# DarylFernandes99/custom-yolo-implmentation

Measured on AMD Instinct MI355X. Metric: images/sec (640x640 bf16), higher is better.
Workload: dtype bf16; 1 GPU; preset s (width 32..512, depth 1) 640x640 train step (fwd+DFL/QFL loss+bwd+grad sync+AdamW), COCO-80 synthetic, 32 img/GPU; global_batch=32, parallelism=dp1, hip_graph=True, optimizer_in_graph=True, deterministic_mode=False

## Files before the change

### custom-yolo-implmentation_amd/csrc/loss.hip

```cpp
#include "common.h"

namespace {

constexpr int REG = 16;
constexpr float QEPS = 1e-12f;

struct LossDims {
    int N, A, nc;
    float lambda_dfl, lambda_cls;
};

template <typename T>
__device__ __forceinline__ void decode_block(const LossDims& d, int block, const T* __restrict__ preds, const T* __restrict__ anchors,
                                             const T* __restrict__ strides, float4* __restrict__ pbox) {
    long i = block * (long)blockDim.x + threadIdx.x;
    if (i >= (long)d.N * d.A) return;
    int a = (int)(i % d.A);
    long n = i / d.A;
    const T* p = preds + n * (long)(4 * REG + d.nc) * d.A + a;
    float e[4];
#pragma unroll
    for (int s = 0; s < 4; ++s) {
        float x[REG], mx = -INFINITY;
#pragma unroll
        for (int b = 0; b < REG; ++b) { x[b] = to_f<T>(p[(long)(s * REG + b) * d.A]); mx = fmaxf(mx, x[b]); }
        float sum = 0.f;
#pragma unroll
        for (int b = 0; b < REG; ++b) { x[b] = expf(x[b] - mx); sum += x[b]; }
        float ex = 0.f;
#pragma unroll
        for (int b = 0; b < REG; ++b) ex += (x[b] / sum) * (float)b;
        e[s] = ex;
    }
    float ax = to_f<T>(anchors[a]), ay = to_f<T>(anchors[d.A + a]), st = to_f<T>(strides[a]);
    float x1 = (ax - e[0]) * st, y1 = (ay - e[1]) * st, x2 = (ax + e[2]) * st, y2 = (ay + e[3]) * st;
    pbox[i] = make_float4((x1 + x2) / 2.f, (y1 + y2) / 2.f, x2 - x1, y2 - y1);
}

__device__ __forceinline__ int assign_wave(int A, const float4* __restrict__ pb, const float* __restrict__ gt, int j, int lane) {
    const float gx = gt[j * 5 + 0], gy = gt[j * 5 + 1];
    const float an = __fadd_rn(__fmul_rn(gx, gx), __fmul_rn(gy, gy));
    const float m2x = -2.f * gx, m2y = -2.f * gy;
    float best = INFINITY;
    int bi = 0x7fffffff;
    auto consider = [&](int a, const float4& b) {
        float bn = __fadd_rn(__fmul_rn(b.x, b.x), __fmul_rn(b.y, b.y));
        float acc = __fmul_rn(m2x, b.x);
        acc = __fmaf_rn(m2y, b.y, acc);
        acc = __fadd_rn(an, acc);
        acc = __fadd_rn(bn, acc);
        float dist = __fsqrt_rn(fmaxf(acc, 0.f));
// ... 37 lines not shown
    float dpos = -2.f * om * ls + om * om / (s + QEPS);
    float dneg = 2.f * s * l1 - s * s / (1.f - s + QEPS);
    dx = -(t * dpos + (1.f - t) * dneg) * s * om;
}

__device__ __forceinline__ void qfl_elem0(float x, float& val, float& dx) {
    float s = sigm(x);
    float l1 = logf(1.f - s + QEPS);
    float om = 1.f - s;
    val = -(s * s * l1);
    float dneg = 2.f * s * l1 - s * s / (1.f - s + QEPS);
    dx = -dneg * s * om;
}

template <typename T, int V>
__device__ __forceinline__ void dense_block(const LossDims& d, int block, int nblk, const T* __restrict__ preds, T* __restrict__ dpreds,
                                            float coef, double* __restrict__ partial, const float* __restrict__ grad_scale) {
    __shared__ float red[4];
    if (grad_scale) coef *= *grad_scale;
    const int Cp = 4 * REG + d.nc;
    const int P = d.nc * (d.A / V), Z = 4 * REG * (d.A / V);
    const int nthr = nblk * 256, gtid = block * 256 + threadIdx.x;
    constexpr int U = 4;
    float lsum = 0.f;
    const long per_img = (long)Cp * d.A;
    for (long i0 = gtid; i0 < (long)d.N * P; i0 += (long)nthr * U) {
        pack_t<T, V> raw[U];
        long eo[U];
#pragma unroll
        for (int u = 0; u < U; ++u) {
            const long idx = i0 + (long)u * nthr;
            const long ic = idx < (long)d.N * P ? idx : i0;
            const int n = (int)(ic / P), off = (int)(ic - (long)n * P);
            eo[u] = n * per_img + (long)4 * REG * d.A + (long)off * V;
            raw[u] = load_raw<T, V>(preds + eo[u]);
        }
#pragma unroll
        for (int u = 0; u < U; ++u) {
            if (i0 + (long)u * nthr >= (long)d.N * P) break;
            float x[V], g[V];
            unpack<T, V>(raw[u], x);
#pragma unroll
            for (int e = 0; e < V; ++e) {
                float v, dx;
                qfl_elem0(x[e], v, dx);
                lsum += v;
                g[e] = dx * coef;
            }
            if (dpreds) store_pack<T, V>(dpreds + eo[u], g);
        }
    }
    if (dpreds) {
        float z[V];
#pragma unroll
        for (int k = 0; k < V; ++k) z[k] = 0.f;
        for (long idx = gtid; idx < (long)d.N * Z; idx += nthr) {
            const int n = (int)(idx / Z), off = (int)(idx - (long)n * Z);
            store_pack<T, V>(dpreds + n * per_img + (long)off * V, z);
        }
    }
    lsum = wave_sum(lsum);
    if ((threadIdx.x & 63) == 0) red[threadIdx.x >> 6] = lsum;
    __syncthreads();
    if (threadIdx.x == 0) partial[block] = (double)red[0] + red[1] + red[2] + red[3];
}

template <typename T, int V>
__global__ __launch_bounds__(256) void k_front(LossDims d, int DB, int nblk, const T* __restrict__ preds, const T* __restrict__ anchors,
                                               const T* __restrict__ strides, float4* __restrict__ pbox, T* __restrict__ dpreds,
                                               float coef, double* __restrict__ partial, const float* __restrict__ grad_scale,
                                               unsigned int* __restrict__ ticket) {
    if (blockIdx.x == 0 && threadIdx.x == 0) *ticket = 0u;
    if ((int)blockIdx.x < DB) decode_block<T>(d, blockIdx.x, preds, anchors, strides, pbox);
    else dense_block<T, V>(d, (int)blockIdx.x - DB, nblk, preds, dpreds, coef, partial, grad_scale);
}

__device__ void finish_scalars(const LossDims& d, const double* partial, int nblk, const double* img_dfl, const double* img_cls_fix,
                               float* __restrict__ out);

template <typename T>
__global__ __launch_bounds__(256) void k_back(LossDims d, const T* __restrict__ preds, T* __restrict__ dpreds,
                                              const T* __restrict__ anchors, const T* __restrict__ strides,
                                              const float4* __restrict__ pbox, const float* __restrict__ gt,
                                              const int* __restrict__ gt_off, const int* __restrict__ idx,
                                              double* __restrict__ img_dfl, double* __restrict__ img_cls_fix,
                                              const float* __restrict__ grad_scale, const double* __restrict__ partial, int nblk,
                                              unsigned int* __restrict__ ticket, float* __restrict__ out) {
    __shared__ double w_dfl[4], w_cls[4];
    __shared__ unsigned int my_ticket;
    const float gsc = grad_scale ? *grad_scale : 1.f;
    const int n = blockIdx.x, lane = threadIdx.x & 63, wave = threadIdx.x >> 6;
    const int g0 = gt_off[n], M = gt_off[n + 1] - g0;

    const int Cp = 4 * REG + d.nc;
    const T* pn = preds + (long)n * Cp * d.A;
    T* dn = dpreds ? dpreds + (long)n * Cp * d.A : nullptr;
    const int side = lane >> 4, bin = lane & 15;
    const float cdfl = d.lambda_dfl / (float)d.N * 0.25f / (float)(M > 0 ? M : 1);
    const float ccls = d.lambda_cls / (float)d.N / (float)d.A;
    double acc_dfl = 0.0, acc_cls = 0.0;

    constexpr int PF = 40;
    const float4* pbn = pbox + (long)n * d.A;
    float2 pf[PF];
#pragma unroll
    for (int u = 0; u < PF; ++u) {
        const int a = threadIdx.x + u * 256;
        pf[u] = (dn && a < d.A) ? *reinterpret_cast<const float2*>(pbn + a) : make_float2(0.f, 0.f);
    }

    for (int j = wave; j < M; j += 4) {
        const int a = idx[g0 + j];
        bool owner = true;
        for (int q = 0; q < j; ++q) owner &= (idx[g0 + q] != a);
        if (!owner) continue;
        float x = to_f<T>(pn[(long)lane * d.A + a]);
        float mx = x;
#pragma unroll
        for (int o = 8; o > 0; o >>= 1) mx = fmaxf(mx, __shfl_xor(mx, o, 64));
        float ex = expf(x - mx), sum = ex;
#pragma unroll
        for (int o = 8; o > 0; o >>= 1) sum += __shfl_xor(sum, o, 64);
        float p = ex / sum, lse = mx + logf(sum);
        float ev = p * (float)bin;
#pragma unroll
        for (int o = 8; o > 0; o >>= 1) ev += __shfl_xor(ev, o, 64);
        const float ax = to_f<T>(anchors[a]), ay = to_f<T>(anchors[d.A + a]), st = to_f<T>(strides[a]);
        const float4 pb = pbox[(long)n * d.A + a];
        float gacc = 0.f;
        int winner = -1;
        for (int q = j; q < M; ++q)
// ... 12 lines not shown
            float contrib = (bin == lo ? wl * (lse - x) : 0.f) + (bin == lo + 1 ? wr * (lse - x) : 0.f);
            float side_loss = contrib;
#pragma unroll
            for (int o = 8; o > 0; o >>= 1) side_loss += __shfl_xor(side_loss, o, 64);
            float all_sides = side_loss + __shfl_xor(side_loss, 16, 64);
            all_sides += __shfl_xor(all_sides, 32, 64);
            if (lane == 0) acc_dfl += (double)all_sides * 0.25 / (double)M;
            gacc += cdfl * (p - (bin == lo ? wl : 0.f) - (bin == lo + 1 ? wr : 0.f));
            const float X1 = pb.x - pb.z / 2.f, Y1 = pb.y - pb.w / 2.f, X2 = pb.x + pb.z / 2.f, Y2 = pb.w + pb.y / 2.f;
            const float iwr = fminf(X2, gx2) - fmaxf(X1, gx1), ihr = fminf(Y2, gy2) - fmaxf(Y1, gy1);
            const float iw = fmaxf(iwr, 0.f), ih = fmaxf(ihr, 0.f);
            const float inter = iw * ih;
            const float a1 = (X2 - X1) * (Y2 - Y1), a2 = (gx2 - gx1) * (gy2 - gy1);
            const float den = a1 + a2 - inter + 1e-6f;
            const float iou = inter / den;
            const float xc = to_f<T>(pn[(long)(4 * REG + cls) * d.A + a]);
            const float sc = sigm(xc);
            const float omc = 1.f - sc;
            const float giou = ccls * -(omc * omc * logf(sc + QEPS) - sc * sc * logf(1.f - sc + QEPS));
            const float mX2 = X2 < gx2 ? 1.f : (X2 == gx2 ? 0.5f : 0.f), mX1 = X1 > gx1 ? 1.f : (X1 == gx1 ? 0.5f : 0.f);
            const float mY2 = Y2 < gy2 ? 1.f : (Y2 == gy2 ? 0.5f : 0.f), mY1 = Y1 > gy1 ? 1.f : (Y1 == gy1 ? 0.5f : 0.f);
            const float pw = iwr >= 0.f ? 1.f : 0.f, ph = ihr >= 0.f ? 1.f : 0.f;
            const float dI_X2 = ih * pw * mX2, dI_X1 = -ih * pw * mX1, dI_Y2 = iw * ph * mY2, dI_Y1 = -iw * ph * mY1;
            const float dA_X2 = (Y2 - Y1), dA_X1 = -(Y2 - Y1), dA_Y2 = (X2 - X1), dA_Y1 = -(X2 - X1);
            const float kI = 1.f / den + inter / (den * den), kA = inter / (den * den);
            const float dX1 = giou * (kI * dI_X1 - kA * dA_X1), dX2 = giou * (kI * dI_X2 - kA * dA_X2);
            const float dY1 = giou * (kI * dI_Y1 - kA * dA_Y1), dY2 = giou * (kI * dI_Y2 - kA * dA_Y2);
            const float dcx = dX1 + dX2, dw = (dX2 - dX1) / 2.f, dcy = dY1 + dY2 / 2.f, dh = dY2 - dY1 / 2.f;
            const float dx1 = dcx / 2.f - dw, dx2 = dcx / 2.f + dw, dy1 = dcy / 2.f - dh, dy2 = dcy / 2.f + dh;
            const float gs = side == 0 ? -st * dx1 : side == 1 ? -st * dy1 : side == 2 ? st * dx2 : st * dy2;
            gacc += gs * p * ((float)bin - ev);
            if (q == winner && lane == 0) {
                float v0, g0_, v1, g1_;
                qfl_elem(xc, 0.f, v0, g0_);
                qfl_elem(xc, iou, v1, g1_);
                acc_cls += (double)v1 - (double)v0;
                if (dn) dn[(long)(4 * REG + cls) * d.A + a] = from_f<T>(g1_ * ccls * gsc);
            }
        }
        if (dn) dn[(long)lane * d.A + a] = from_f<T>(gacc * gsc);
    }
    if (dn) {
        auto poison = [&](int a, float cx, float cy) {
            const bool bx = cx != cx, by = cy != cy;
            if (!(bx || by)) return;
            for (int c = 0; c < 4 * REG; ++c)
                if (((c >> 4) & 1) ? by : bx) dn[(long)c * d.A + a] = from_f<T>(NAN);
        };
#pragma unroll
        for (int u = 0; u < PF; ++u) poison(threadIdx.x + u * 256, pf[u].x, pf[u].y);
        for (int a = threadIdx.x + PF * 256; a < d.A; a += 256) poison(a, pbn[a].x, pbn[a].y);
    }
    if (lane == 0) { w_dfl[wave] = acc_dfl; w_cls[wave] = acc_cls; }
    __syncthreads();
    if (threadIdx.x == 0) {
        img_dfl[n] = w_dfl[0] + w_dfl[1] + w_dfl[2] + w_dfl[3];
        img_cls_fix[n] = w_cls[0] + w_cls[1] + w_cls[2] + w_cls[3];
        __threadfence();
        my_ticket = atomicAdd(ticket, 1u);
    }
    __syncthreads();
    if (my_ticket != (unsigned)d.N - 1u || wave != 0) return;
// ... 28 lines not shown
    double mean_cls = cls / (double)d.A / (double)d.N, mean_dfl = dfl / (double)d.N;
    out[0] = (float)(d.lambda_dfl * mean_dfl + d.lambda_cls * mean_cls);
    out[1] = (float)mean_dfl;
    out[2] = (float)mean_cls;
}

template <typename T>
__global__ void k_scale(T* __restrict__ x, long n, const float* __restrict__ s) {
    const float f = *s;
    for (long i = blockIdx.x * (long)blockDim.x + threadIdx.x; i < n; i += (long)gridDim.x * blockDim.x)
        x[i] = from_f<T>(to_f<T>(x[i]) * f);
}

constexpr int DENSE_BLOCKS = 2048;

}

extern "C" {

size_t yolo_loss_workspace_bytes(int N, int A, int G) {
    size_t b = (size_t)N * A * 16;
    b += ((size_t)(G > 0 ? G : 1) * 4 + 15) / 16 * 16;
    b += (size_t)(DENSE_BLOCKS + 2 * N) * 8;
    b += 16;
    return b;
}

int yolo_loss_dfl_qfl(const void* preds, const void* anchors, const void* strides, int dtype, int N, int nc, int A,
                      const float* gt, const int* gt_off, const int* gt_img, int G, float lambda_dfl,
                      float lambda_cls, void* dpreds, float* out, void* workspace, const float* grad_scale, hipStream_t st) {
    if (N < 1) return YOLO_ERR_ARG;
    LossDims d{N, A, nc, lambda_dfl, lambda_cls};
    char* ws = (char*)workspace;
    float4* pbox = (float4*)ws;
    ws += (size_t)N * A * 16;
    int* idx = (int*)ws;
    ws += ((size_t)(G > 0 ? G : 1) * 4 + 15) / 16 * 16;
    double* partial = (double*)ws;
    double* img_dfl = partial + DENSE_BLOCKS;
    double* img_fix = img_dfl + N;
    unsigned int* ticket = (unsigned int*)(img_fix + N);
    const long NA = (long)N * A;
    const long elems = NA * (64 + nc);
    const float coef = lambda_cls / (float)N / (float)A;
    const int DB = ceil_div(NA, 256);
    YOLO_DISPATCH_T(dtype, {
        constexpr int VV = vec_of<T>::N;
        bool vec = (A % VV == 0) && ((uintptr_t)preds % 16 == 0) && (!dpreds || (uintptr_t)dpreds % 16 == 0);
        int nblk = (int)((elems / (vec ? VV : 1) + 255) / 256);
        if (nblk > DENSE_BLOCKS) nblk = DENSE_BLOCKS;
        if (nblk < 1) nblk = 1;
        if (vec) hipLaunchKernelGGL((k_front<T, VV>), dim3(DB + nblk), dim3(256), 0, st, d, DB, nblk, (const T*)preds, (const T*)anchors,
                                    (const T*)strides, pbox, (T*)dpreds, coef, partial, grad_scale, ticket);
        else hipLaunchKernelGGL((k_front<T, 1>), dim3(DB + nblk), dim3(256), 0, st, d, DB, nblk, (const T*)preds, (const T*)anchors,
                                (const T*)strides, pbox, (T*)dpreds, coef, partial, grad_scale, ticket);
        if (G > 0) hipLaunchKernelGGL(k_assign, dim3(ceil_div(G, 4)), dim3(256), 0, st, A, pbox, gt, gt_img, gt_off, N, idx);
        hipLaunchKernelGGL((k_back<T>), dim3(N), dim3(256), 0, st, d, (const T*)preds, (T*)dpreds, (const T*)anchors,
                           (const T*)strides, pbox, gt, gt_off, idx, img_dfl, img_fix, grad_scale, partial, nblk, ticket, out);
    });
    return YOLO_LAUNCH_CHECK();
}

int yolo_scale_inplace(void* x, long n, int dtype, const float* scale_dev, hipStream_t st) {
    long b = (n + 255) / 256;
    if (b > 4096) b = 4096;
    if (b < 1) b = 1;
    YOLO_DISPATCH_T(dtype, hipLaunchKernelGGL((k_scale<T>), dim3((int)b), dim3(256), 0, st, (T*)x, n, scale_dev));
    return YOLO_LAUNCH_CHECK();
}

}
```

### custom-yolo-implmentation_amd/src/hipops/functions.py

```python
import os

import torch

from . import ops
from .lib import ACT_IDENTITY, ACT_SILU

_LOWP = (torch.bfloat16, torch.float16)


def compute_dtype(x, w):
    dev = x.device.type
    if torch.is_autocast_enabled(dev):
        return torch.get_autocast_dtype(dev)
    if w.dtype in _LOWP:
        return w.dtype
    return x.dtype if x.dtype in (torch.float32,) + _LOWP else torch.float32


def _as_nhwc(t, dtype):
    return t if (t.dtype == dtype and ops.is_nhwc(t)) else ops.to_nhwc(t, dtype)


def _f32(t):
    return t if t.dtype == torch.float32 else t.float()
# ... 627 lines not shown
        ctx.save_for_backward(qkv, o, lse)
        return o, vp

    @staticmethod
    def backward(ctx, d_o, d_vp):
        heads, dk, dh, scale = ctx.cfg
        qkv, o, lse = ctx.saved_tensors
        T = qkv.dtype
        if d_o is None:
            d_o = ops.zero_(ops.new_nhwc(*o.shape, T, o.device))
        d_o = _as_nhwc(d_o, T)
        d_vp = _as_nhwc(d_vp, T) if d_vp is not None else None
        return ops.attn_bwd(qkv, o, d_o, d_vp, lse, heads, dk, dh, scale), None, None, None, None


class HeadPack(torch.autograd.Function):

    @staticmethod
    def forward(ctx, *branches):
        T = branches[0].dtype
        branches = [_as_nhwc(b, T) for b in branches]
        n = branches[0].shape[0]
        levels = [(branches[i], branches[i + 1]) for i in range(0, len(branches), 2)]
        no = levels[0][0].shape[1] + levels[0][1].shape[1]
        m = sum(b.shape[2] * b.shape[3] for b, _ in levels)
        preds = torch.empty((n, no, m), dtype=T, device=branches[0].device)
        meta, m_off, c_offs, m_offs = [], 0, [], []
        for box, cls in levels:
            h, w = box.shape[2], box.shape[3]
            c_offs += [0, box.shape[1]]
            m_offs += [m_off, m_off]
            meta.append((box.shape[1], cls.shape[1], h, w, m_off))
            m_off += h * w
        ops.head_group(branches, preds, c_offs, m_offs, True)
        ctx.meta = meta
        return preds

    @staticmethod
    def backward(ctx, dpreds):
        dpreds = dpreds.contiguous()
        n = dpreds.shape[0]
        grads, c_offs, m_offs = [], [], []
        for cb, cc, h, w, m_off in ctx.meta:
            grads += [ops.new_nhwc(n, cb, h, w, dpreds.dtype, dpreds.device), ops.new_nhwc(n, cc, h, w, dpreds.dtype, dpreds.device)]
            c_offs += [0, cb]
            m_offs += [m_off, m_off]
        ops.head_group(grads, dpreds, c_offs, m_offs, False)
        return tuple(grads)


UNIT_LOSS_SEED = False
LOSS_SCALE = None


class DflQflLoss(torch.autograd.Function):

    @staticmethod
    def forward(ctx, preds, anchors, strides, packed, nc, lambda_dfl, lambda_cls):
        gt, gt_off, gt_img, n_gt = packed
        want = ctx.needs_input_grad[0]
        out, dpreds, _ = ops.loss_fwd_bwd(preds.contiguous(), anchors, strides, gt, gt_off, gt_img, n_gt, nc,
                                          lambda_dfl, lambda_cls, want, LOSS_SCALE if want else None)
        ctx.dpreds = dpreds
        ctx.mark_non_differentiable(out)
        return out[0].clone(), out

    @staticmethod
    def backward(ctx, g_total, _g_scalars):
        dpreds = ctx.dpreds
        ctx.dpreds = None
        if dpreds is None:
            return (None,) * 7
        if not UNIT_LOSS_SEED:
            ops.scale_inplace(dpreds, g_total.reshape(1).float())
        return dpreds, None, None, None, None, None, None
```

### custom-yolo-implmentation_amd/src/hipops/ops.py

```python
import os

import torch

from . import lib

ALGO = int(os.environ.get("YOLO_HIP_CONV_ALGO", "0"))

_DT = {torch.float32: lib.F32, torch.bfloat16: lib.BF16, torch.float16: lib.F16}


def dt(t):
    try:
        return _DT[t.dtype if isinstance(t, torch.Tensor) else t]
    except KeyError:
        raise RuntimeError(f"unsupported dtype {t}")


def _stream(t):
    if not t.is_cuda:
        raise RuntimeError("yolo_hip ops need tensors on the GPU: the product path has no CPU fallback "
                           "(the CPU oracle lives under oracle/ and is test infrastructure)")
    return _raw_stream(t.device.index)


# ... 520 lines not shown
    lib.status(rc, "yolo_attn_fwd_nograd")
    return o, vp


def attn_bwd(qkv, o, d_o, d_vp, stash, heads, dk, dh, scale):
    n, cq, h, w, ld = geom(qkv)
    t = h * w
    dqkv = new_nhwc(n, cq, h, w, qkv.dtype, qkv.device)
    ws = torch.empty(lib.query("yolo_attn_workspace_bytes_for", n, t, heads, dk, dh, dt(qkv)), dtype=torch.uint8, device=qkv.device)
    lib.call("yolo_attn_bwd", _p(qkv), ld, _p(o), geom(o)[4], _p(d_o), geom(d_o)[4], _p(d_vp),
             geom(d_vp)[4] if d_vp is not None else 0, _p(stash), _p(ws), _p(dqkv), cq, n, t, heads, dk, dh,
             float(scale), dt(qkv), _stream(qkv))
    return dqkv


def loss_fwd_bwd(preds, anchors, strides, gt, gt_off, gt_img, n_gt, nc, lambda_dfl, lambda_cls, want_grad, grad_scale=None):
    assert grad_scale is None or (grad_scale.dtype == torch.float32 and grad_scale.is_cuda)
    n, cp, a = preds.shape
    assert preds.is_contiguous() and cp == 64 + nc
    anchors = anchors.to(preds.dtype).contiguous()
    strides = strides.to(preds.dtype).contiguous()
    ws = torch.empty(lib.query("yolo_loss_workspace_bytes", n, a, n_gt), dtype=torch.uint8, device=preds.device)
    out = _f32(3, preds.device)
    dpreds = torch.empty_like(preds) if want_grad else None
    lib.call("yolo_loss_dfl_qfl", _p(preds), _p(anchors), _p(strides), dt(preds), n, nc, a, _p(gt), _p(gt_off),
             _p(gt_img), n_gt, float(lambda_dfl), float(lambda_cls), _p(dpreds), _p(out), _p(ws), _p(grad_scale), _stream(preds))
    return out, dpreds, ws


def _f32c(t):
    if t.dtype != torch.float32 or not t.is_contiguous():
        raise RuntimeError("the stand-alone loss helpers take contiguous fp32 tensors")
    return t


def bbox_iou(b1, b2, g=None):
    m = b1.shape[0]
    _f32c(b1), _f32c(b2)
# ... 139 lines not shown
```

### custom-yolo-implmentation_amd/src/model/head.py

```python
import math
from typing import List

import torch
from torch import nn

from src.hipops import functions as F_
from src.model.model_blocks import DFL, Conv
from src.utils.model_utils import make_anchors_cached


class Head(nn.Module):
    anchors = torch.empty(0)
    strides = torch.empty(0)

    def __init__(self, nc: int = 1, filters: List[int] = []):
        super().__init__()
        self.ch = 16
        self.nc = nc
        self.nl = len(filters)
        self.no = nc + self.ch * 4
        self.stride = torch.zeros(self.nl)
        box = max(64, filters[0] // 4)
        cls = max(80, filters[0], self.nc)
        self.dfl = DFL(self.ch)
# ... 28 lines not shown
            dev = x[0].device
            cur, side = torch.cuda.current_stream(dev), F_.side_stream(dev)
            side.wait_stream(cur)
            F_.FWD_STREAM = side
            try:
                cls_outs = [self._branch(self.cls[i], xc[i], links[i]) for i in range(self.nl)]
            finally:
                F_.FWD_STREAM = None
            box_outs = [self._branch(self.box[i], xb[i], links[i]) for i in range(self.nl)]
            cur.wait_stream(side)
            outs = [o for pair in zip(box_outs, cls_outs) for o in pair]
        else:
            outs = []
            for i in range(self.nl):
                outs += [self._branch(self.box[i], xb[i], links[i]), self._branch(self.cls[i], xc[i], links[i])]
        preds = F_.HeadPack.apply(*outs)
        shapes = tuple((int(o.shape[2]), int(o.shape[3])) for o in outs[::2])
        anchors, strides = make_anchors_cached(shapes, tuple(float(s) for s in self.stride), preds.dtype, preds.device)
        return preds, anchors, strides
```

### custom-yolo-implmentation_amd/src/training/graph_step.py

```python
import gc
import os

import torch
import torch.distributed as dist

from src.hipops import functions as F_
from src.hipops import lib
from src.hipops import ops


class GradBuckets:

    ALIGN = 16

    def __init__(self, stage_params, comm_dtype):
        self.stage_params = [[p for p in ps if p.requires_grad] for ps in stage_params]
        self.comm_dtype = comm_dtype
        self.flats = None
        self.plans = {}
        self._pending = []

    def _ensure_flats(self):
        if self.flats is not None:
            return
# ... 107 lines not shown

    def _lazy(self, device):
        return device.type == "cuda" and os.environ.get("YOLO_LAZY_JOIN", "1") == "1" and all(p.grad is None for p in self.params)

    def _stage_a(self, images, packed):
        dev = images.device
        cut = {}
        if self.staged:
            def at_cut(feats):
                cut["out"] = list(feats)
                cut["leaf"] = [t.detach().requires_grad_(True) for t in feats]
                return cut["leaf"]
            self.model.stage_cut = at_cut
        F_.LAZY_WGRAD_JOIN = self._lazy(dev)
        F_.LOSS_SCALE = self.amp.scale if self.amp is not None else None
        try:
            with torch.autocast(dev.type, dtype=self.amp_dtype, enabled=self.amp_dtype is not None):
                preds, anchors, strides = self.model(images)
                loss, ld = self.criterion(preds, packed, anchors, strides)
            F_.LOSS_SCALE = None
            F_.UNIT_LOSS_SEED = type(loss.grad_fn).__name__ == "DflQflLossBackward" and os.environ.get("YOLO_UNIT_SEED", "1") == "1"
            loss.backward()
        except BaseException:
            F_.LAZY_WGRAD_JOIN = False
            self._cut = None
            raise
        finally:
            F_.UNIT_LOSS_SEED = False
            F_.LOSS_SCALE = None
            if self.staged:
                self.model.stage_cut = None
            if not self.staged:
                F_.LAZY_WGRAD_JOIN = False
            if dev.type == "cuda":
# ... 186 lines not shown
```

### include/yolo_hip.h

```cpp
#ifndef YOLO_HIP_H
#define YOLO_HIP_H
#include <stddef.h>
#include <stdint.h>

#ifdef __cplusplus
extern "C" {
#endif

#ifndef __HIP__
typedef struct ihipStream_t* hipStream_t;
#endif

#define YOLO_F32 0
#define YOLO_BF16 1
#define YOLO_F16 2
#define YOLO_ERR_ARG 1001
#define YOLO_ERR_DTYPE 1002
#define YOLO_ACT_IDENTITY 0
#define YOLO_ACT_SILU 1

long yolo_abi_hash(void);

int yolo_memset0(void* p, size_t bytes, hipStream_t st);
int yolo_ncm_to_nhwc(const void* src, int src_dtype, long sn, long sc, long off, void* dst, int dst_dtype, int ld, int N, int C, int HW, hipStream_t st);
// ... 77 lines not shown
int yolo_maxpool5_fwd(const void* x, int ldx, void* out, int ldo, uint8_t* idx, int N, int H, int W, int C, int dtype, hipStream_t st);
int yolo_maxpool5_bwd(const void* dout, int ldd, const uint8_t* idx, void* dx, int ldx, int N, int H, int W, int C, int accumulate, int dtype, hipStream_t st);
int yolo_upsample2x_fwd(const void* x, int ldx, void* out, int ldo, int N, int H, int W, int C, int dtype, hipStream_t st);
int yolo_upsample2x_bwd(const void* dout, int ldd, void* dx, int ldx, int N, int H, int W, int C, int accumulate, int dtype, hipStream_t st);

size_t yolo_attn_stash_bytes(int N, int T_, int heads, int dtype);
size_t yolo_attn_workspace_bytes(int N, int T_, int heads, int dtype);
size_t yolo_attn_stash_bytes_for(int N, int T, int heads, int dk, int dh, int dtype);
size_t yolo_attn_workspace_bytes_for(int N, int T, int heads, int dk, int dh, int dtype);
int yolo_attn_fwd(const void* qkv, int ldq, void* o, int ldo, void* vp, int ldv, void* stash, void* ws, int N, int T_, int heads, int dk, int dh, float scale, int dtype, hipStream_t st);
int yolo_attn_fwd_nograd(const void* qkv, int ldq, void* o, int ldo, void* vp, int ldv, int N, int T_, int heads, int dk, int dh, float scale, int dtype, hipStream_t st);
int yolo_attn_bwd(const void* qkv, int ldq, const void* o, int ldo, const void* d_o, int lddo, const void* d_vp, int lddv, const void* stash, void* ws, void* dqkv, int lddq, int N, int T_, int heads, int dk, int dh, float scale, int dtype, hipStream_t st);

size_t yolo_loss_workspace_bytes(int N, int A, int G);
int yolo_loss_dfl_qfl(const void* preds, const void* anchors, const void* strides, int dtype, int N, int nc, int A, const float* gt, const int* gt_off, const int* gt_img, int G, float lambda_dfl, float lambda_cls, void* dpreds, float* out, void* workspace, const float* grad_scale, hipStream_t st);

int yolo_bbox_iou(const float* box1, const float* box2, int M, float* iou, const float* g, float* db1, float* db2, hipStream_t st);
int yolo_quality_focal_loss(const float* pred, const float* target, int M, int C, float beta, float* out, const float* g, float* dpred, float* dtarget, hipStream_t st);
int yolo_distribution_focal_loss(const float* pred_dist, const float* target_val, int M, int C, float* out, const float* g, float* dpred, float* dtarget, hipStream_t st);

int yolo_head_decode(const void* preds, const void* anchors, const void* strides, void* y, int N, int nc, int A, int dtype, hipStream_t st);
int yolo_dfl_expect(const void* x, void* y, int B, int A, int dtype, hipStream_t st);
int yolo_nms_capacity(int M, int nc, int multi_label);
size_t yolo_nms_workspace_bytes(int bs, int M, int nc, int multi_label);
int yolo_nms(const void* y, int dtype, int bs, int nc, int M, float conf_thres, float iou_thres, const int* classes, int n_classes, int agnostic, int multi_label, int max_det, float* out, int* out_count, int* status, void* workspace, hipStream_t st);

size_t yolo_val_workspace_bytes(int N, int M, int top_k);
int yolo_val_select(const void* y, int dtype, int N, int nc, int M, float conf, int top_k, float* out, int* out_count, void* workspace, hipStream_t st);
int yolo_val_match(const float* pred, const int* count, int N, int top_k, const float* gt, const int* gt_off, double iou_thr, int nc, int skip_empty_gt, long long* counters, int* status, hipStream_t st);

// ... 20 lines not shown
```

Before: 3117 images/s.

## Compute DFL/QFL loss directly on per-level NHWC head outputs, skipping HeadPack

```diff
diff --git a/custom-yolo-implmentation_amd/csrc/loss.hip b/custom-yolo-implmentation_amd/csrc/loss.hip
--- a/custom-yolo-implmentation_amd/csrc/loss.hip
+++ b/custom-yolo-implmentation_amd/csrc/loss.hip
@@ -10,31 +10,121 @@
     float lambda_dfl, lambda_cls;
 };
 
+constexpr int MAXL = 4;
+
 template <typename T>
-__device__ __forceinline__ void decode_block(const LossDims& d, int block, const T* __restrict__ preds, const T* __restrict__ anchors,
+struct PackedLay {
+    const T* preds;
+    T* dpreds;
+    int A, Cp;
+    __device__ __forceinline__ bool grad() const { return dpreds != nullptr; }
+    __device__ __forceinline__ long step() const { return A; }
+    __device__ __forceinline__ const T* box(int n, int a) const { return preds + (long)n * Cp * A + a; }
+    __device__ __forceinline__ const T* cls(int n, int a) const { return preds + ((long)n * Cp + 4 * REG) * A + a; }
+    __device__ __forceinline__ T* dbox(int n, int a) const { return dpreds + (long)n * Cp * A + a; }
+    __device__ __forceinline__ T* dcls(int n, int a) const { return dpreds + ((long)n * Cp + 4 * REG) * A + a; }
+};
+
+template <typename T>
+struct LevelLay {
+    const T* pb[MAXL];
+    const T* pc[MAXL];
+    T* gb[MAXL];
+    T* gc[MAXL];
+    int ldb[MAXL], ldc[MAXL], lgb[MAXL], lgc[MAXL], hw[MAXL], off[MAXL];
+    int N;
+    template <typename P>
+    __device__ __forceinline__ P* at(P* const (&ptr)[MAXL], const int (&ld)[MAXL], int n, int a) const {
+        P* p = ptr[0];
+        int l_ = ld[0], h = hw[0], o = 0;
+#pragma unroll
+        for (int l = 1; l < MAXL; ++l)
+            if (a >= off[l]) { p = ptr[l]; l_ = ld[l]; h = hw[l]; o = off[l]; }
+        return p + ((long)n * h + (a - o)) * l_;
+    }
+    template <typename P>
+    __device__ __forceinline__ P* row(P* const (&ptr)[MAXL], const int (&ld)[MAXL], int r) const {
+        P* p = ptr[0];
+        int l_ = ld[0], o = 0;
+#pragma unroll
+        for (int l = 1; l < MAXL; ++l)
+            if (r >= N * off[l]) { p = ptr[l]; l_ = ld[l]; o = N * off[l]; }
+        return p + (long)(r - o) * l_;
+    }
+    __device__ __forceinline__ bool grad() const { return gb[0] != nullptr; }
+    __device__ __forceinline__ long step() const { return 1; }
+    __device__ __forceinline__ const T* box(int n, int a) const { return at(pb, ldb, n, a); }
+    __device__ __forceinline__ const T* cls(int n, int a) const { return at(pc, ldc, n, a); }
+    __device__ __forceinline__ T* dbox(int n, int a) const { return at(gb, lgb, n, a); }
+    __device__ __forceinline__ T* dcls(int n, int a) const { return at(gc, lgc, n, a); }
+};
+
+__device__ __forceinline__ float side_expect(float (&x)[REG]) {
+    float mx = -INFINITY;
+#pragma unroll
+    for (int b = 0; b < REG; ++b) mx = fmaxf(mx, x[b]);
+    float sum = 0.f;
+#pragma unroll
+    for (int b = 0; b < REG; ++b) { x[b] = expf(x[b] - mx); sum += x[b]; }
+    float ex = 0.f;
+#pragma unroll
+    for (int b = 0; b < REG; ++b) ex += (x[b] / sum) * (float)b;
+    return ex;
+}
+
+template <typename T>
+__device__ __forceinline__ float4 decode_box(const float (&e)[4], int a, int A, const T* __restrict__ anchors, const T* __restrict__ strides) {
+    float ax = to_f<T>(anchors[a]), ay = to_f<T>(anchors[A + a]), st = to_f<T>(strides[a]);
+    float x1 = (ax - e[0]) * st, y1 = (ay - e[1]) * st, x2 = (ax + e[2]) * st, y2 = (ay + e[3]) * st;
+    return make_float4((x1 + x2) / 2.f, (y1 + y2) / 2.f, x2 - x1, y2 - y1);
+}
+
+template <typename T, int V>
+__device__ __forceinline__ void decode_block(const LossDims& d, int block, const PackedLay<T>& lay, const T* __restrict__ anchors,
                                              const T* __restrict__ strides, float4* __restrict__ pbox) {
     long i = block * (long)blockDim.x + threadIdx.x;
     if (i >= (long)d.N * d.A) return;
     int a = (int)(i % d.A);
     long n = i / d.A;
-    const T* p = preds + n * (long)(4 * REG + d.nc) * d.A + a;
+    const T* p = lay.box((int)n, a);
     float e[4];
 #pragma unroll
     for (int s = 0; s < 4; ++s) {
-        float x[REG], mx = -INFINITY;
-#pragma unroll
-        for (int b = 0; b < REG; ++b) { x[b] = to_f<T>(p[(long)(s * REG + b) * d.A]); mx = fmaxf(mx, x[b]); }
-        float sum = 0.f;
-#pragma unroll
-        for (int b = 0; b < REG; ++b) { x[b] = expf(x[b] - mx); sum += x[b]; }
-        float ex = 0.f;
-#pragma unroll
-        for (int b = 0; b < REG; ++b) ex += (x[b] / sum) * (float)b;
-        e[s] = ex;
-    }
-    float ax = to_f<T>(anchors[a]), ay = to_f<T>(anchors[d.A + a]), st = to_f<T>(strides[a]);
-    float x1 = (ax - e[0]) * st, y1 = (ay - e[1]) * st, x2 = (ax + e[2]) * st, y2 = (ay + e[3]) * st;
-    pbox[i] = make_float4((x1 + x2) / 2.f, (y1 + y2) / 2.f, x2 - x1, y2 - y1);
+        float x[REG];
+#pragma unroll
+        for (int b = 0; b < REG; ++b) x[b] = to_f<T>(p[(long)(s * REG + b) * d.A]);
+        e[s] = side_expect(x);
+    }
+    pbox[i] = decode_box<T>(e, a, d.A, anchors, strides);
+}
+
+template <typename T, int V>
+__device__ __forceinline__ void decode_block(const LossDims& d, int block, const LevelLay<T>& lay, const T* __restrict__ anchors,
+                                             const T* __restrict__ strides, float4* __restrict__ pbox) {
+    const long NA = (long)d.N * d.A;
+    long i = (block * (long)blockDim.x + threadIdx.x) >> 2;
+    const int s = threadIdx.x & 3;
+    const bool live = i < NA;
+    if (!live) i = NA - 1;
+    const int a = (int)(i % d.A), n = (int)(i / d.A);
+    const T* p = lay.box(n, a) + s * REG;
+    pack_t<T, V> raw[REG / V];
+#pragma unroll
+    for (int k = 0; k < REG / V; ++k) raw[k] = load_raw<T, V>(p + k * V);
+    float x[REG];
+#pragma unroll
+    for (int k = 0; k < REG / V; ++k) {
+        float t[V];
+        unpack<T, V>(raw[k], t);
+#pragma unroll
+        for (int b = 0; b < V; ++b) x[k * V + b] = t[b];
+    }
+    const float ex = side_expect(x);
+    const int l0 = (threadIdx.x & 63) & ~3;
+    float e[4];
+#pragma unroll
+    for (int k = 0; k < 4; ++k) e[k] = __shfl(ex, l0 + k, 64);
+    if (live && s == 0) pbox[i] = decode_box<T>(e, a, d.A, anchors, strides);
 }
 
 __device__ __forceinline__ int assign_wave(int A, const float4* __restrict__ pb, const float* __restrict__ gt, int j, int lane) {
@@ -102,9 +192,72 @@
 }
 
 template <typename T, int V>
-__device__ __forceinline__ void dense_block(const LossDims& d, int block, int nblk, const T* __restrict__ preds, T* __restrict__ dpreds,
+__device__ __forceinline__ void dense_packet(const pack_t<T, V>& raw, float coef, float& lsum, float (&g)[V]) {
+    float x[V];
+    unpack<T, V>(raw, x);
+#pragma unroll
+    for (int e = 0; e < V; ++e) {
+        float v, dx;
+        qfl_elem0(x[e], v, dx);
+        lsum += v;
+        g[e] = dx * coef;
+    }
+}
+
+__device__ __forceinline__ void dense_partial(float lsum, int block, double* __restrict__ partial) {
+    __shared__ float red[4];
+    lsum = wave_sum(lsum);
+    if ((threadIdx.x & 63) == 0) red[threadIdx.x >> 6] = lsum;
+    __syncthreads();
+    if (threadIdx.x == 0) partial[block] = (double)red[0] + red[1] + red[2] + red[3];
+}
+
+template <typename T, int V>
+__device__ __forceinline__ void dense_block(const LossDims& d, int block, int nblk, const LevelLay<T>& lay, float coef,
+                                            double* __restrict__ partial, const float* __restrict__ grad_scale) {
+    if (grad_scale) coef *= *grad_scale;
+    const bool grad = lay.grad();
+    const int PR = d.nc / V, ZR = 4 * REG / V;
+    const int P = d.N * d.A * PR, Z = d.N * d.A * ZR;
+    const int nthr = nblk * 256, gtid = block * 256 + threadIdx.x;
+    constexpr int U = 4;
+    float lsum = 0.f;
+    for (long i0 = gtid; i0 < P; i0 += (long)nthr * U) {
+        pack_t<T, V> raw[U];
+        int r[U], k[U];
+#pragma unroll
+        for (int u = 0; u < U; ++u) {
+            const long idx = i0 + (long)u * nthr;
+            const int ic = (int)(idx < P ? idx : i0);
+            r[u] = ic / PR;
+            k[u] = (ic - r[u] * PR) * V;
+            raw[u] = load_raw<T, V>(lay.row(lay.pc, lay.ldc, r[u]) + k[u]);
+        }
+#pragma unroll
+        for (int u = 0; u < U; ++u) {
+            if (i0 + (long)u * nthr >= P) break;
+            float g[V];
+            dense_packet<T, V>(raw[u], coef, lsum, g);
+            if (grad) store_pack<T, V>(lay.row(lay.gc, lay.lgc, r[u]) + k[u], g);
+        }
+    }
+    if (grad) {
+        float z[V];
+#pragma unroll
+        for (int k = 0; k < V; ++k) z[k] = 0.f;
+        for (long idx = gtid; idx < Z; idx += nthr) {
+            const int r = (int)idx / ZR, k = ((int)idx - r * ZR) * V;
+            store_pack<T, V>(lay.row(lay.gb, lay.lgb, r) + k, z);
+        }
+    }
+    dense_partial(lsum, block, partial);
+}
+
+template <typename T, int V>
+__device__ __forceinline__ void dense_block(const LossDims& d, int block, int nblk, const PackedLay<T>& lay,
                                             float coef, double* __restrict__ partial, const float* __restrict__ grad_scale) {
-    __shared__ float red[4];
+    const T* __restrict__ preds = lay.preds;
+    T* __restrict__ dpreds = lay.dpreds;
     if (grad_scale) coef *= *grad_scale;
     const int Cp = 4 * REG + d.nc;
     const int P = d.nc * (d.A / V), Z = 4 * REG * (d.A / V);
@@ -126,15 +279,8 @@
 #pragma unroll
         for (int u = 0; u < U; ++u) {
             if (i0 + (long)u * nthr >= (long)d.N * P) break;
-            float x[V], g[V];
-            unpack<T, V>(raw[u], x);
-#pragma unroll
-            for (int e = 0; e < V; ++e) {
-                float v, dx;
-                qfl_elem0(x[e], v, dx);
-                lsum += v;
-                g[e] = dx * coef;
-            }
+            float g[V];
+            dense_packet<T, V>(raw[u], coef, lsum, g);
             if (dpreds) store_pack<T, V>(dpreds + eo[u], g);
         }
     }
@@ -147,28 +293,24 @@
             store_pack<T, V>(dpreds + n * per_img + (long)off * V, z);
         }
     }
-    lsum = wave_sum(lsum);
-    if ((threadIdx.x & 63) == 0) red[threadIdx.x >> 6] = lsum;
-    __syncthreads();
-    if (threadIdx.x == 0) partial[block] = (double)red[0] + red[1] + red[2] + red[3];
-}
-
-template <typename T, int V>
-__global__ __launch_bounds__(256) void k_front(LossDims d, int DB, int nblk, const T* __restrict__ preds, const T* __restrict__ anchors,
-                                               const T* __restrict__ strides, float4* __restrict__ pbox, T* __restrict__ dpreds,
+    dense_partial(lsum, block, partial);
+}
+
+template <typename T, int V, typename Lay>
+__global__ __launch_bounds__(256) void k_front(LossDims d, int DB, int nblk, Lay lay, const T* __restrict__ anchors,
+                                               const T* __restrict__ strides, float4* __restrict__ pbox,
                                                float coef, double* __restrict__ partial, const float* __restrict__ grad_scale,
                                                unsigned int* __restrict__ ticket) {
     if (blockIdx.x == 0 && threadIdx.x == 0) *ticket = 0u;
-    if ((int)blockIdx.x < DB) decode_block<T>(d, blockIdx.x, preds, anchors, strides, pbox);
-    else dense_block<T, V>(d, (int)blockIdx.x - DB, nblk, preds, dpreds, coef, partial, grad_scale);
+    if ((int)blockIdx.x < DB) decode_block<T, V>(d, blockIdx.x, lay, anchors, strides, pbox);
+    else dense_block<T, V>(d, (int)blockIdx.x - DB, nblk, lay, coef, partial, grad_scale);
 }
 
 __device__ void finish_scalars(const LossDims& d, const double* partial, int nblk, const double* img_dfl, const double* img_cls_fix,
                                float* __restrict__ out);
 
-template <typename T>
-__global__ __launch_bounds__(256) void k_back(LossDims d, const T* __restrict__ preds, T* __restrict__ dpreds,
-                                              const T* __restrict__ anchors, const T* __restrict__ strides,
+template <typename T, typename Lay>
+__global__ __launch_bounds__(256) void k_back(LossDims d, Lay lay, const T* __restrict__ anchors, const T* __restrict__ strides,
                                               const float4* __restrict__ pbox, const float* __restrict__ gt,
                                               const int* __restrict__ gt_off, const int* __restrict__ idx,
                                               double* __restrict__ img_dfl, double* __restrict__ img_cls_fix,
@@ -180,9 +322,8 @@
     const int n = blockIdx.x, lane = threadIdx.x & 63, wave = threadIdx.x >> 6;
     const int g0 = gt_off[n], M = gt_off[n + 1] - g0;
 
-    const int Cp = 4 * REG + d.nc;
-    const T* pn = preds + (long)n * Cp * d.A;
-    T* dn = dpreds ? dpreds + (long)n * Cp * d.A : nullptr;
+    const bool dn = lay.grad();
+    const long cs = lay.step();
     const int side = lane >> 4, bin = lane & 15;
     const float cdfl = d.lambda_dfl / (float)d.N * 0.25f / (float)(M > 0 ? M : 1);
     const float ccls = d.lambda_cls / (float)d.N / (float)d.A;
@@ -202,7 +343,9 @@
         bool owner = true;
         for (int q = 0; q < j; ++q) owner &= (idx[g0 + q] != a);
         if (!owner) continue;
-        float x = to_f<T>(pn[(long)lane * d.A + a]);
+        const T* pba = lay.box(n, a);
+        const T* pca = lay.cls(n, a);
+        float x = to_f<T>(pba[(long)lane * cs]);
         float mx = x;
 #pragma unroll
         for (int o = 8; o > 0; o >>= 1) mx = fmaxf(mx, __shfl_xor(mx, o, 64));
@@ -245,7 +388,7 @@
             const float a1 = (X2 - X1) * (Y2 - Y1), a2 = (gx2 - gx1) * (gy2 - gy1);
             const float den = a1 + a2 - inter + 1e-6f;
             const float iou = inter / den;
-            const float xc = to_f<T>(pn[(long)(4 * REG + cls) * d.A + a]);
+            const float xc = to_f<T>(pca[(long)cls * cs]);
             const float sc = sigm(xc);
             const float omc = 1.f - sc;
             const float giou = ccls * -(omc * omc * logf(sc + QEPS) - sc * sc * logf(1.f - sc + QEPS));
@@ -266,17 +409,18 @@
                 qfl_elem(xc, 0.f, v0, g0_);
                 qfl_elem(xc, iou, v1, g1_);
                 acc_cls += (double)v1 - (double)v0;
-                if (dn) dn[(long)(4 * REG + cls) * d.A + a] = from_f<T>(g1_ * ccls * gsc);
+                if (dn) lay.dcls(n, a)[(long)cls * cs] = from_f<T>(g1_ * ccls * gsc);
             }
         }
-        if (dn) dn[(long)lane * d.A + a] = from_f<T>(gacc * gsc);
+        if (dn) lay.dbox(n, a)[(long)lane * cs] = from_f<T>(gacc * gsc);
     }
     if (dn) {
         auto poison = [&](int a, float cx, float cy) {
             const bool bx = cx != cx, by = cy != cy;
             if (!(bx || by)) return;
+            T* da = lay.dbox(n, a);
             for (int c = 0; c < 4 * REG; ++c)
-                if (((c >> 4) & 1) ? by : bx) dn[(long)c * d.A + a] = from_f<T>(NAN);
+                if (((c >> 4) & 1) ? by : bx) da[(long)c * cs] = from_f<T>(NAN);
         };
 #pragma unroll
         for (int u = 0; u < PF; ++u) poison(threadIdx.x + u * 256, pf[u].x, pf[u].y);
@@ -335,6 +479,38 @@
 
 constexpr int DENSE_BLOCKS = 2048;
 
+struct LossWs {
+    float4* pbox;
+    int* idx;
+    double *partial, *img_dfl, *img_fix;
+    unsigned int* ticket;
+    LossWs(void* workspace, int N, int A, int G) {
+        char* ws = (char*)workspace;
+        pbox = (float4*)ws;
+        ws += (size_t)N * A * 16;
+        idx = (int*)ws;
+        ws += ((size_t)(G > 0 ? G : 1) * 4 + 15) / 16 * 16;
+        partial = (double*)ws;
+        img_dfl = partial + DENSE_BLOCKS;
+        img_fix = img_dfl + N;
+        ticket = (unsigned int*)(img_fix + N);
+    }
+};
+
+template <typename T, int V, typename Lay>
+void launch_loss(const LossDims& d, const Lay& lay, int DB, long packets, const LossWs& w, const void* anchors, const void* strides,
+                 const float* gt, const int* gt_off, const int* gt_img, int G, const float* grad_scale, float* out, hipStream_t st) {
+    const float coef = d.lambda_cls / (float)d.N / (float)d.A;
+    int nblk = (int)((packets + 255) / 256);
+    if (nblk > DENSE_BLOCKS) nblk = DENSE_BLOCKS;
+    if (nblk < 1) nblk = 1;
+    hipLaunchKernelGGL((k_front<T, V, Lay>), dim3(DB + nblk), dim3(256), 0, st, d, DB, nblk, lay, (const T*)anchors,
+                       (const T*)strides, w.pbox, coef, w.partial, grad_scale, w.ticket);
+    if (G > 0) hipLaunchKernelGGL(k_assign, dim3(ceil_div(G, 4)), dim3(256), 0, st, d.A, w.pbox, gt, gt_img, gt_off, d.N, w.idx);
+    hipLaunchKernelGGL((k_back<T, Lay>), dim3(d.N), dim3(256), 0, st, d, lay, (const T*)anchors, (const T*)strides, w.pbox, gt,
+                       gt_off, w.idx, w.img_dfl, w.img_fix, grad_scale, w.partial, nblk, w.ticket, out);
+}
+
 }
 
 extern "C" {
@@ -352,32 +528,62 @@
                       float lambda_cls, void* dpreds, float* out, void* workspace, const float* grad_scale, hipStream_t st) {
     if (N < 1) return YOLO_ERR_ARG;
     LossDims d{N, A, nc, lambda_dfl, lambda_cls};
-    char* ws = (char*)workspace;
-    float4* pbox = (float4*)ws;
-    ws += (size_t)N * A * 16;
-    int* idx = (int*)ws;
-    ws += ((size_t)(G > 0 ? G : 1) * 4 + 15) / 16 * 16;
-    double* partial = (double*)ws;
-    double* img_dfl = partial + DENSE_BLOCKS;
-    double* img_fix = img_dfl + N;
-    unsigned int* ticket = (unsigned int*)(img_fix + N);
+    const LossWs w(workspace, N, A, G);
     const long NA = (long)N * A;
     const long elems = NA * (64 + nc);
-    const float coef = lambda_cls / (float)N / (float)A;
     const int DB = ceil_div(NA, 256);
     YOLO_DISPATCH_T(dtype, {
         constexpr int VV = vec_of<T>::N;
+        const PackedLay<T> lay{(const T*)preds, (T*)dpreds, A, 64 + nc};
         bool vec = (A % VV == 0) && ((uintptr_t)preds % 16 == 0) && (!dpreds || (uintptr_t)dpreds % 16 == 0);
-        int nblk = (int)((elems / (vec ? VV : 1) + 255) / 256);
-        if (nblk > DENSE_BLOCKS) nblk = DENSE_BLOCKS;
-        if (nblk < 1) nblk = 1;
-        if (vec) hipLaunchKernelGGL((k_front<T, VV>), dim3(DB + nblk), dim3(256), 0, st, d, DB, nblk, (const T*)preds, (const T*)anchors,
-                                    (const T*)strides, pbox, (T*)dpreds, coef, partial, grad_scale, ticket);
-        else hipLaunchKernelGGL((k_front<T, 1>), dim3(DB + nblk), dim3(256), 0, st, d, DB, nblk, (const T*)preds, (const T*)anchors,
-                                (const T*)strides, pbox, (T*)dpreds, coef, partial, grad_scale, ticket);
-        if (G > 0) hipLaunchKernelGGL(k_assign, dim3(ceil_div(G, 4)), dim3(256), 0, st, A, pbox, gt, gt_img, gt_off, N, idx);
-        hipLaunchKernelGGL((k_back<T>), dim3(N), dim3(256), 0, st, d, (const T*)preds, (T*)dpreds, (const T*)anchors,
-                           (const T*)strides, pbox, gt, gt_off, idx, img_dfl, img_fix, grad_scale, partial, nblk, ticket, out);
+        if (vec) launch_loss<T, VV>(d, lay, DB, elems / VV, w, anchors, strides, gt, gt_off, gt_img, G, grad_scale, out, st);
+        else launch_loss<T, 1>(d, lay, DB, elems, w, anchors, strides, gt, gt_off, gt_img, G, grad_scale, out, st);
+    });
+    return YOLO_LAUNCH_CHECK();
+}
+
+int yolo_loss_dfl_qfl_levels(int L, const void* const* box, const void* const* cls, const int* ld_box, const int* ld_cls,
+                             const int* HWs, const int* a_offs, void* const* dbox, void* const* dcls, const int* ld_dbox,
+                             const int* ld_dcls, const void* anchors, const void* strides, int dtype, int N, int nc, int A,
+                             const float* gt, const int* gt_off, const int* gt_img, int G, float lambda_dfl, float lambda_cls,
+                             float* out, void* workspace, const float* grad_scale, hipStream_t st) {
+    if (N < 1 || nc < 1 || L < 1 || L > MAXL) return YOLO_ERR_ARG;
+    const bool grad = dbox != nullptr;
+    if (grad && dcls == nullptr) return YOLO_ERR_ARG;
+    long sum = 0;
+    for (int l = 0; l < L; ++l) {
+        if (HWs[l] < 1 || a_offs[l] != sum || ld_box[l] < 64 || ld_cls[l] < nc || !box[l] || !cls[l]) return YOLO_ERR_ARG;
+        if (grad && (ld_dbox[l] < 64 || ld_dcls[l] < nc || !dbox[l] || !dcls[l])) return YOLO_ERR_ARG;
+        sum += HWs[l];
+    }
+    const long NA = (long)N * A;
+    if (sum != A || NA * (nc > 64 ? nc : 64) >= (1L << 31)) return YOLO_ERR_ARG;
+    LossDims d{N, A, nc, lambda_dfl, lambda_cls};
+    const LossWs w(workspace, N, A, G);
+    const int DB = ceil_div(4 * NA, 256);
+    YOLO_DISPATCH_T(dtype, {
+        constexpr int VV = vec_of<T>::N;
+        LevelLay<T> lay;
+        bool vec = nc % VV == 0;
+        for (int l = 0; l < MAXL; ++l) {
+            const bool on = l < L;
+            lay.pb[l] = on ? (const T*)box[l] : nullptr;
+            lay.pc[l] = on ? (const T*)cls[l] : nullptr;
+            lay.gb[l] = on && grad ? (T*)dbox[l] : nullptr;
+            lay.gc[l] = on && grad ? (T*)dcls[l] : nullptr;
+            lay.ldb[l] = on ? ld_box[l] : 0;
+            lay.ldc[l] = on ? ld_cls[l] : 0;
+            lay.lgb[l] = on && grad ? ld_dbox[l] : 0;
+            lay.lgc[l] = on && grad ? ld_dcls[l] : 0;
+            lay.hw[l] = on ? HWs[l] : 0;
+            lay.off[l] = on ? a_offs[l] : A;
+            if (!on) continue;
+            vec = vec && ld_box[l] % VV == 0 && ld_cls[l] % VV == 0 && (uintptr_t)box[l] % 16 == 0 && (uintptr_t)cls[l] % 16 == 0;
+            if (grad) vec = vec && ld_dbox[l] % VV == 0 && ld_dcls[l] % VV == 0 && (uintptr_t)dbox[l] % 16 == 0 && (uintptr_t)dcls[l] % 16 == 0;
+        }
+        lay.N = N;
+        if (vec) launch_loss<T, VV>(d, lay, DB, NA * ((64 + nc) / VV), w, anchors, strides, gt, gt_off, gt_img, G, grad_scale, out, st);
+        else launch_loss<T, 1>(d, lay, DB, NA * (64 + nc), w, anchors, strides, gt, gt_off, gt_img, G, grad_scale, out, st);
     });
     return YOLO_LAUNCH_CHECK();
 }
diff --git a/custom-yolo-implmentation_amd/src/hipops/functions.py b/custom-yolo-implmentation_amd/src/hipops/functions.py
--- a/custom-yolo-implmentation_amd/src/hipops/functions.py
+++ b/custom-yolo-implmentation_amd/src/hipops/functions.py
@@ -665,10 +665,37 @@
         return ops.attn_bwd(qkv, o, d_o, d_vp, lse, heads, dk, dh, scale), None, None, None, None
 
 
+HEAD_LEVELS_ENABLED = os.environ.get("YOLO_HEAD_LEVELS", "1") == "1"
+HEAD_LEVELS = False
+LEVEL_LINK = None
+
+
+class LevelLink:
+    __slots__ = ("branches", "ptr", "shape", "grads")
+
+    def __init__(self, branches, preds):
+        self.branches, self.ptr, self.shape, self.grads = branches, preds.data_ptr(), tuple(preds.shape), None
+
+    def stands_for(self, preds):
+        return preds.data_ptr() == self.ptr and tuple(preds.shape) == self.shape and preds.is_contiguous()
+
+
+def take_level_link(preds):
+    global LEVEL_LINK
+    link, LEVEL_LINK = LEVEL_LINK, None
+    if link is None:
+        return None
+    if not link.stands_for(preds):
+        raise RuntimeError("the head left its outputs in level layout (functions.HEAD_LEVELS) but the loss received another "
+                           "tensor than the head's preds: the unfilled preds must go straight into DflQflLoss")
+    return link
+
+
 class HeadPack(torch.autograd.Function):
 
     @staticmethod
     def forward(ctx, *branches):
+        global LEVEL_LINK
         T = branches[0].dtype
         branches = [_as_nhwc(b, T) for b in branches]
         n = branches[0].shape[0]
@@ -676,6 +703,10 @@
         no = levels[0][0].shape[1] + levels[0][1].shape[1]
         m = sum(b.shape[2] * b.shape[3] for b, _ in levels)
         preds = torch.empty((n, no, m), dtype=T, device=branches[0].device)
+        ctx.link = None
+        if HEAD_LEVELS and HEAD_LEVELS_ENABLED and preds.is_cuda and len(levels) <= 4 and levels[0][0].shape[1] == 64:
+            ctx.link = LEVEL_LINK = LevelLink(branches, preds)
+            return preds
         meta, m_off, c_offs, m_offs = [], 0, [], []
         for box, cls in levels:
             h, w = box.shape[2], box.shape[3]
@@ -689,6 +720,11 @@
 
     @staticmethod
     def backward(ctx, dpreds):
+        if ctx.link is not None:
+            grads, ctx.link.grads = ctx.link.grads, None
+            if grads is None:
+                raise RuntimeError("HeadPack.backward on the level path without the level gradients of DflQflLoss")
+            return tuple(grads)
         dpreds = dpreds.contiguous()
         n = dpreds.shape[0]
         grads, c_offs, m_offs = [], [], []
@@ -710,6 +746,17 @@
     def forward(ctx, preds, anchors, strides, packed, nc, lambda_dfl, lambda_cls):
         gt, gt_off, gt_img, n_gt = packed
         want = ctx.needs_input_grad[0]
+        link = take_level_link(preds) if LEVEL_LINK is not None else None
+        if link is not None:
+            out, grads, _ = ops.loss_fwd_bwd(preds, anchors, strides, gt, gt_off, gt_img, n_gt, nc, lambda_dfl, lambda_cls,
+                                             want, LOSS_SCALE if want else None, levels=link.branches)
+            link.branches = None
+            link.grads = grads
+            ctx.dpreds = preds.new_empty(1).expand(preds.shape) if want else None
+            ctx.on_levels = True
+            ctx.mark_non_differentiable(out)
+            return out[0].clone(), out
+        ctx.on_levels = False
         out, dpreds, _ = ops.loss_fwd_bwd(preds.contiguous(), anchors, strides, gt, gt_off, gt_img, n_gt, nc,
                                           lambda_dfl, lambda_cls, want, LOSS_SCALE if want else None)
         ctx.dpreds = dpreds
@@ -722,6 +769,10 @@
         ctx.dpreds = None
         if dpreds is None:
             return (None,) * 7
+        if ctx.on_levels:
+            if not UNIT_LOSS_SEED:
+                raise RuntimeError("the level path of the loss is only taken where the backward seed is exactly 1 (UNIT_LOSS_SEED)")
+            return dpreds, None, None, None, None, None, None
         if not UNIT_LOSS_SEED:
             ops.scale_inplace(dpreds, g_total.reshape(1).float())
         return dpreds, None, None, None, None, None, None
diff --git a/custom-yolo-implmentation_amd/src/hipops/ops.py b/custom-yolo-implmentation_amd/src/hipops/ops.py
--- a/custom-yolo-implmentation_amd/src/hipops/ops.py
+++ b/custom-yolo-implmentation_amd/src/hipops/ops.py
@@ -558,7 +558,12 @@
     return dqkv
 
 
-def loss_fwd_bwd(preds, anchors, strides, gt, gt_off, gt_img, n_gt, nc, lambda_dfl, lambda_cls, want_grad, grad_scale=None):
+def level_index(shapes, level, pixel, channel):
+    return channel, sum(h * w for h, w in shapes[:level]) + pixel
+
+
+def loss_fwd_bwd(preds, anchors, strides, gt, gt_off, gt_img, n_gt, nc, lambda_dfl, lambda_cls, want_grad, grad_scale=None,
+                 levels=None, level_grads=None):
     assert grad_scale is None or (grad_scale.dtype == torch.float32 and grad_scale.is_cuda)
     n, cp, a = preds.shape
     assert preds.is_contiguous() and cp == 64 + nc
@@ -566,6 +571,28 @@
     strides = strides.to(preds.dtype).contiguous()
     ws = torch.empty(lib.query("yolo_loss_workspace_bytes", n, a, n_gt), dtype=torch.uint8, device=preds.device)
     out = _f32(3, preds.device)
+    if levels is not None:
+        import ctypes
+        k = len(levels) // 2
+        gs = [geom(t) for t in levels]
+        assert len(levels) == 2 * k and 1 <= k <= 4 and all(t.dtype == preds.dtype for t in levels)
+        assert all(g[0] == n for g in gs) and all(gs[2 * i][1:4] == (64,) + gs[2 * i + 1][2:4] and gs[2 * i + 1][1] == nc for i in range(k))
+        grads = None
+        if want_grad:
+            grads = level_grads if level_grads is not None else [new_nhwc(*g[:4], preds.dtype, preds.device) for g in gs]
+            gg = [geom(t) for t in grads]
+            assert len(grads) == 2 * k and all(x[:4] == y[:4] for x, y in zip(gg, gs)) and all(t.dtype == preds.dtype for t in grads)
+        hws = [g[2] * g[3] for g in gs[::2]]
+        offs = [sum(hws[:i]) for i in range(k)]
+        assert sum(hws) == a
+        vp, i32 = ctypes.c_void_p * k, ctypes.c_int * k
+        lib.call("yolo_loss_dfl_qfl_levels", k, vp(*[t.data_ptr() for t in levels[::2]]), vp(*[t.data_ptr() for t in levels[1::2]]),
+                 i32(*[g[4] for g in gs[::2]]), i32(*[g[4] for g in gs[1::2]]), i32(*hws), i32(*offs),
+                 vp(*[t.data_ptr() for t in grads[::2]]) if grads else None, vp(*[t.data_ptr() for t in grads[1::2]]) if grads else None,
+                 i32(*[g[4] for g in gg[::2]]) if grads else None, i32(*[g[4] for g in gg[1::2]]) if grads else None,
+                 _p(anchors), _p(strides), dt(preds), n, nc, a, _p(gt), _p(gt_off), _p(gt_img), n_gt, float(lambda_dfl),
+                 float(lambda_cls), _p(out), _p(ws), _p(grad_scale), _stream(preds))
+        return out, grads, ws
     dpreds = torch.empty_like(preds) if want_grad else None
     lib.call("yolo_loss_dfl_qfl", _p(preds), _p(anchors), _p(strides), dt(preds), n, nc, a, _p(gt), _p(gt_off),
              _p(gt_img), n_gt, float(lambda_dfl), float(lambda_cls), _p(dpreds), _p(out), _p(ws), _p(grad_scale), _stream(preds))
diff --git a/custom-yolo-implmentation_amd/src/model/head.py b/custom-yolo-implmentation_amd/src/model/head.py
--- a/custom-yolo-implmentation_amd/src/model/head.py
+++ b/custom-yolo-implmentation_amd/src/model/head.py
@@ -66,7 +66,11 @@
             outs = []
             for i in range(self.nl):
                 outs += [self._branch(self.box[i], xb[i], links[i]), self._branch(self.cls[i], xc[i], links[i])]
-        preds = F_.HeadPack.apply(*outs)
+        levels, F_.HEAD_LEVELS = F_.HEAD_LEVELS, F_.HEAD_LEVELS and self.training and not self._forward_hooks
+        try:
+            preds = F_.HeadPack.apply(*outs)
+        finally:
+            F_.HEAD_LEVELS = levels
         shapes = tuple((int(o.shape[2]), int(o.shape[3])) for o in outs[::2])
         anchors, strides = make_anchors_cached(shapes, tuple(float(s) for s in self.stride), preds.dtype, preds.device)
         return preds, anchors, strides
diff --git a/custom-yolo-implmentation_amd/src/training/graph_step.py b/custom-yolo-implmentation_amd/src/training/graph_step.py
--- a/custom-yolo-implmentation_amd/src/training/graph_step.py
+++ b/custom-yolo-implmentation_amd/src/training/graph_step.py
@@ -7,6 +7,7 @@
 from src.hipops import functions as F_
 from src.hipops import lib
 from src.hipops import ops
+from src.model.losses import YoloDFLQFLoss
 
 
 class GradBuckets:
@@ -145,10 +146,16 @@
             self.model.stage_cut = at_cut
         F_.LAZY_WGRAD_JOIN = self._lazy(dev)
         F_.LOSS_SCALE = self.amp.scale if self.amp is not None else None
+        F_.HEAD_LEVELS = dev.type == "cuda" and type(self.criterion) is YoloDFLQFLoss and not self.model._forward_hooks \
+            and os.environ.get("YOLO_UNIT_SEED", "1") == "1"
         try:
             with torch.autocast(dev.type, dtype=self.amp_dtype, enabled=self.amp_dtype is not None):
-                preds, anchors, strides = self.model(images)
-                loss, ld = self.criterion(preds, packed, anchors, strides)
+                try:
+                    preds, anchors, strides = self.model(images)
+                    loss, ld = self.criterion(preds, packed, anchors, strides)
+                finally:
+                    F_.HEAD_LEVELS = False
+                    F_.LEVEL_LINK = None
             F_.LOSS_SCALE = None
             F_.UNIT_LOSS_SEED = type(loss.grad_fn).__name__ == "DflQflLossBackward" and os.environ.get("YOLO_UNIT_SEED", "1") == "1"
             loss.backward()
diff --git a/include/yolo_hip.h b/include/yolo_hip.h
--- a/include/yolo_hip.h
+++ b/include/yolo_hip.h
@@ -115,6 +115,7 @@
 
 size_t yolo_loss_workspace_bytes(int N, int A, int G);
 int yolo_loss_dfl_qfl(const void* preds, const void* anchors, const void* strides, int dtype, int N, int nc, int A, const float* gt, const int* gt_off, const int* gt_img, int G, float lambda_dfl, float lambda_cls, void* dpreds, float* out, void* workspace, const float* grad_scale, hipStream_t st);
+int yolo_loss_dfl_qfl_levels(int L, const void* const* box, const void* const* cls, const int* ld_box, const int* ld_cls, const int* HWs, const int* a_offs, void* const* dbox, void* const* dcls, const int* ld_dbox, const int* ld_dcls, const void* anchors, const void* strides, int dtype, int N, int nc, int A, const float* gt, const int* gt_off, const int* gt_img, int G, float lambda_dfl, float lambda_cls, float* out, void* workspace, const float* grad_scale, hipStream_t st);
 
 int yolo_bbox_iou(const float* box1, const float* box2, int M, float* iou, const float* g, float* db1, float* db2, hipStream_t st);
 int yolo_quality_focal_loss(const float* pred, const float* target, int M, int C, float beta, float* out, const float* g, float* dpred, float* dtarget, hipStream_t st);
```

New measurement: 3133 images/s, median of 6. About the same (+0.5%).
